# thygate/stable-diffusion-webui-depthmap-script

Measured on NVIDIA H100. Metric: images/sec, higher is better.
Workload: dtype fp16

## Files before the change

stable-diffusion-webui-depthmap-script_b200/csrc/attention_wgmma.cu:

```cuda
#include <cuda.h>
#include <cuda_fp16.h>
#include <math.h>

#include "common.cuh"
#include "tc_common.cuh"

namespace dm {
using namespace tc;

__device__ __forceinline__ float ex2_approx(float x) {
    float y;
    asm("ex2.approx.ftz.f32 %0, %1;" : "=f"(y) : "f"(x));
    return y;
}

int make_tmap_2d(CUtensorMap *tm, const void *ptr, uint64_t rows, uint64_t cols, uint64_t ld, uint32_t box_rows, uint32_t box_cols);

struct AttnParams {
    int B, N, H;
    int C;
    float scale_log2e;
    const __half *bias;
    int bias_ld;
    __half *out;
    const float *rel_table;
    int nrd, gh, gw;
    int sub_stride;
};

constexpr int AT_BQ = 128, AT_BKV = 128, AT_D = 64, AT_STAGES = 2;
constexpr int AT_THREADS = 384;
constexpr int AT_Q_BYTES = AT_BQ * AT_D * 2;
constexpr int AT_KV_BYTES = AT_BKV * AT_D * 2;
constexpr int AT_K_OFF = AT_Q_BYTES;
constexpr int AT_V_OFF = AT_K_OFF + AT_STAGES * AT_KV_BYTES;
constexpr int AT_BAR_OFF = AT_V_OFF + AT_STAGES * AT_KV_BYTES;
constexpr int AT_TAB_OFF = AT_BAR_OFF + 64;
constexpr int AT_SMEM_MAX = 227 * 1024;
constexpr int AT_STAGERS = 96;

static inline int relpos_sub_stride(int gh, int gw) {
    const int span = gh < (AT_BQ - 1) / gw + 2 ? gh : (AT_BQ - 1) / gw + 2;
    return ((2 * span - 1) * (2 * gw - 1) + 1 + 3) & ~3;
}

template <int BIAS_MODE>
__global__ void __launch_bounds__(AT_THREADS, 1) attention_wgmma_kernel(const __grid_constant__ CUtensorMap tmQKV, AttnParams p) {
    extern __shared__ __align__(1024) uint8_t smem_raw[];
    uint8_t *sQ = smem_raw, *sK = smem_raw + AT_K_OFF, *sV = smem_raw + AT_V_OFF;
    uint64_t *bars = reinterpret_cast<uint64_t *>(smem_raw + AT_BAR_OFF);
    uint64_t *q_full = bars, *kv_full = bars + 1, *kv_empty = bars + 1 + AT_STAGES;
    float *s_tab = reinterpret_cast<float *>(smem_raw + AT_TAB_OFF);
    int *s_koff = reinterpret_cast<int *>(s_tab + AT_STAGES * p.sub_stride);

    const int warp = threadIdx.x >> 5, lane = threadIdx.x & 31;
    const int q0 = blockIdx.x * AT_BQ, h = blockIdx.y, b = blockIdx.z;
    const int num_kv = (p.N + AT_BKV - 1) / AT_BKV;
    const int row_base = b * p.N;

    if (threadIdx.x == 0) {
        prefetch_tmap(&tmQKV);
        mbar_init(q_full, 1);
        for (int s = 0; s < AT_STAGES; ++s) {
            mbar_init(&kv_full[s], BIAS_MODE == 2 ? 1 + AT_STAGERS : 1);
            mbar_init(&kv_empty[s], 8);
        }
        fence_barrier_init();
    }
    __syncthreads();

    if (warp < 4) {
        if (threadIdx.x == 0) {
            mbar_arrive_expect_tx(q_full, AT_Q_BYTES);
            tma_load_2d(sQ, &tmQKV, q_full, h * AT_D, row_base + q0);
            for (int j = 0; j < num_kv; ++j) {
                const int s = j % AT_STAGES;
                mbar_wait(&kv_empty[s], ((j / AT_STAGES) & 1) ^ 1);
                mbar_arrive_expect_tx(&kv_full[s], 2 * AT_KV_BYTES);
                tma_load_2d(sK + s * AT_KV_BYTES, &tmQKV, &kv_full[s], p.C + h * AT_D, row_base + j * AT_BKV);
                tma_load_2d(sV + s * AT_KV_BYTES, &tmQKV, &kv_full[s], 2 * p.C + h * AT_D, row_base + j * AT_BKV);
            }
        } else if (BIAS_MODE == 2 && warp >= 1) {
            const int st = threadIdx.x - 32, rw = 2 * p.gw - 1;
            const float *tab = p.rel_table + (size_t)h * p.nrd;
            const int qy_min = (max(q0, 1) - 1) / p.gw, qy_max = (min(q0 + AT_BQ, p.N) - 2) / p.gw;
            for (int j = 0; j < num_kv; ++j) {
                const int s = j % AT_STAGES, kbase = j * AT_BKV;
                const int k_lo = max(kbase, 1), k_hi = min(kbase + AT_BKV, p.N) - 1;
                const int ky_min = (k_lo - 1) / p.gw, ky_max = (k_hi - 1) / p.gw;
                const int lo = (qy_min - ky_max + p.gh - 1) * rw;
                const int cnt = (qy_max - qy_min + ky_max - ky_min + 1) * rw;
                float *sub = s_tab + s * p.sub_stride;
                int *kof = s_koff + s * AT_BKV;
                mbar_wait(&kv_empty[s], ((j / AT_STAGES) & 1) ^ 1);
                for (int i = st; i < cnt; i += AT_STAGERS) sub[i] = __ldg(tab + lo + i);
                if (st == 0) sub[p.sub_stride - 1] = __ldg(tab + p.nrd - 3);
                for (int k = st; k < AT_BKV; k += AT_STAGERS) {
                    const int t = min(max(kbase + k, k_lo), k_hi) - 1;
                    kof[k] = (t / p.gw) * rw + (t % p.gw) + lo;
                }
                mbar_arrive(&kv_full[s]);
            }
        }
        return;
    }

    const int wg = (warp >> 2) - 1, t = lane & 3;
    constexpr float LOG2E = 1.4426950408889634f;
    int qi[2];
    bool q_ok[2];
    const __half *brow[2] = {nullptr, nullptr};
    int rp_base[2] = {0, 0}, rp_mult[2] = {1, 1};
    float rp_k0[2] = {0.f, 0.f};
#pragma unroll
    for (int r = 0; r < 2; ++r) {
        qi[r] = q0 + wg * 64 + (warp & 3) * 16 + (lane >> 2) + 8 * r;
        q_ok[r] = qi[r] < p.N;
        const int qq = q_ok[r] ? qi[r] : 0;
        if (BIAS_MODE == 1) brow[r] = p.bias + ((size_t)h * p.N + qq) * p.bias_ld;
        if (BIAS_MODE == 2) {
            const float *tab = p.rel_table + (size_t)h * p.nrd;
            if (qq == 0) { rp_base[r] = p.sub_stride - 1; rp_mult[r] = 0; rp_k0[r] = __ldg(tab + p.nrd - 1); }
            else {
                const int tt = qq - 1, qy = tt / p.gw, qx = tt % p.gw;
                rp_base[r] = (qy + p.gh - 1) * (2 * p.gw - 1) + (qx + p.gw - 1);
                rp_k0[r] = __ldg(tab + p.nrd - 2);
            }
        }
    }
    float o[32];
#pragma unroll
    for (int i = 0; i < 32; ++i) o[i] = 0.f;
    float m_run[2] = {-INFINITY, -INFINITY}, l_run[2] = {0.f, 0.f};
    const uint64_t qdesc = make_desc_kmajor_sw128(smem_u32(sQ) + wg * (64 * 128));

    mbar_wait(q_full, 0);
    for (int j = 0; j < num_kv; ++j) {
        const int s = j % AT_STAGES;
        const int kbase = j * AT_BKV;
        mbar_wait(&kv_full[s], (j / AT_STAGES) & 1);
        float sc[64];
        const float *sub = s_tab + s * p.sub_stride;
        const int *kof = s_koff + s * AT_BKV;
        const uint64_t kdesc = make_desc_kmajor_sw128(smem_u32(sK + s * AT_KV_BYTES));
        wgmma_fence();
#pragma unroll
        for (int k = 0; k < AT_D / 16; ++k) wgmma_ss<AT_BKV>(sc, qdesc + (uint64_t)(2 * k), kdesc + (uint64_t)(2 * k), k != 0);
        wgmma_commit();
        wgmma_wait<0>();
        float mx[2] = {-INFINITY, -INFINITY};
#pragma unroll
        for (int c = 0; c < AT_BKV / 8; ++c) {
            const int k0 = kbase + 8 * c + 2 * t;
#pragma unroll
            for (int r = 0; r < 2; ++r) {
                float b0 = 0.f, b1 = 0.f;
                if (BIAS_MODE == 1) {
                    const float2 bf = __half22float2(__ldg(reinterpret_cast<const __half2 *>(brow[r] + k0)));
                    b0 = bf.x * LOG2E; b1 = bf.y * LOG2E;
                } else if (BIAS_MODE == 2) {
                    const int2 kk = *reinterpret_cast<const int2 *>(kof + 8 * c + 2 * t);
                    b0 = k0 == 0 ? rp_k0[r] : sub[rp_base[r] - rp_mult[r] * kk.x];
                    b1 = sub[rp_base[r] - rp_mult[r] * kk.y];
                }
                float u0 = fmaf(sc[4 * c + 2 * r], p.scale_log2e, b0), u1 = fmaf(sc[4 * c + 2 * r + 1], p.scale_log2e, b1);
                u0 = k0 < p.N ? u0 : -INFINITY;
                u1 = k0 + 1 < p.N ? u1 : -INFINITY;
                sc[4 * c + 2 * r] = u0; sc[4 * c + 2 * r + 1] = u1;
                mx[r] = fmaxf(mx[r], fmaxf(u0, u1));
            }
        }
        float alpha[2];
#pragma unroll
        for (int r = 0; r < 2; ++r) {
            mx[r] = fmaxf(mx[r], __shfl_xor_sync(0xffffffffu, mx[r], 1));
            mx[r] = fmaxf(mx[r], __shfl_xor_sync(0xffffffffu, mx[r], 2));
            const float m_new = fmaxf(m_run[r], mx[r]);
            alpha[r] = ex2_approx(m_run[r] - m_new);
            m_run[r] = m_new;
        }
        uint32_t pa[AT_BKV / 16][4];
        float ls[2] = {0.f, 0.f};
#pragma unroll
        for (int c = 0; c < AT_BKV / 8; ++c) {
#pragma unroll
            for (int r = 0; r < 2; ++r) {
                const float e0 = ex2_approx(sc[4 * c + 2 * r] - m_run[r]), e1 = ex2_approx(sc[4 * c + 2 * r + 1] - m_run[r]);
                const __half2 h2 = __floats2half2_rn(e0, e1);
                const float2 pr = __half22float2(h2);
                ls[r] += pr.x + pr.y;
                pa[c >> 1][(c & 1) * 2 + r] = *reinterpret_cast<const uint32_t *>(&h2);
            }
        }
#pragma unroll
        for (int r = 0; r < 2; ++r) l_run[r] = fmaf(l_run[r], alpha[r], ls[r]);
#pragma unroll
        for (int c = 0; c < AT_D / 8; ++c) { o[4 * c] *= alpha[0]; o[4 * c + 1] *= alpha[0]; o[4 * c + 2] *= alpha[1]; o[4 * c + 3] *= alpha[1]; }
        const uint32_t sv = smem_u32(sV + s * AT_KV_BYTES);
        wgmma_fence();
#pragma unroll
        for (int k = 0; k < AT_BKV / 16; ++k) wgmma_rs_n64_bt(o, pa[k], make_desc_mnmajor_sw128(sv + k * 16 * 128));
        wgmma_commit();
        wgmma_wait<0>();
        if (lane == 0) mbar_arrive(&kv_empty[s]);
    }
#pragma unroll
    for (int r = 0; r < 2; ++r) {
        float l = l_run[r];
        l += __shfl_xor_sync(0xffffffffu, l, 1);
        l += __shfl_xor_sync(0xffffffffu, l, 2);
        if (!q_ok[r]) continue;
        const float inv = 1.0f / l;
        __half *dst = p.out + (size_t)(row_base + qi[r]) * p.C + h * AT_D + 2 * t;
#pragma unroll
        for (int c = 0; c < AT_D / 8; ++c)
            *reinterpret_cast<__half2 *>(dst + 8 * c) = __floats2half2_rn(o[4 * c + 2 * r] * inv, o[4 * c + 2 * r + 1] * inv);
    }
}

template <int MODE>
static int launch_attn(const CUtensorMap &tm, const AttnParams &p, cudaStream_t stream) {
    const size_t tab = MODE == 2 ? (size_t)AT_STAGES * ((size_t)p.sub_stride * 4 + AT_BKV * 4) : 0;
    if (AT_TAB_OFF + tab > (size_t)AT_SMEM_MAX) { set_error("attention: relative-position window %d x %d too wide for the table sub-windows", p.gh, p.gw); return DM_E_UNSUPPORTED; }
    static PerDeviceFlag configured;
    if (!configured.test_and_set())
        DM_CUDA_CHECK(cudaFuncSetAttribute(attention_wgmma_kernel<MODE>, cudaFuncAttributeMaxDynamicSharedMemorySize, AT_SMEM_MAX));
    dim3 grid((p.N + AT_BQ - 1) / AT_BQ, p.H, p.B);
    attention_wgmma_kernel<MODE><<<grid, AT_THREADS, AT_TAB_OFF + tab, stream>>>(tm, p);
    DM_LAUNCH_CHECK("attention_wgmma_kernel");
    return DM_OK;
}

int attention_f16(const __half *qkv, AttnParams p, cudaStream_t stream, const float *rel_table = nullptr, int nrd = 0, int gh = 0, int gw = 0) {
    if (p.C != p.H * AT_D) { set_error("attention_f16: head_dim must be 64"); return DM_E_UNSUPPORTED; }
    CUtensorMap tm;
    int rc = make_tmap_2d(&tm, qkv, (uint64_t)p.B * p.N, (uint64_t)3 * p.C, (uint64_t)3 * p.C, AT_BQ, AT_D);
    if (rc) return rc;
    if (p.bias && (p.bias_ld % 8 != 0 || p.bias_ld < ((p.N + AT_BKV - 1) / AT_BKV) * AT_BKV)) {
        set_error("attention_f16: bias row pitch must be a multiple of 8 and cover whole 128-key tiles (got %d)", p.bias_ld);
        return DM_E_INVALID;
    }
    p.rel_table = rel_table; p.nrd = nrd; p.gh = gh; p.gw = gw; p.sub_stride = 0;
    if (rel_table) {
        if (gh < 1 || gw < 1 || (long long)gh * gw + 1 != p.N || (long long)nrd != (long long)(2 * gh - 1) * (2 * gw - 1) + 3) {
            set_error("attention_f16: relative-position mode needs N = gh*gw+1 and nrd = (2gh-1)(2gw-1)+3");
            return DM_E_INVALID;
        }
        p.sub_stride = relpos_sub_stride(gh, gw);
        return launch_attn<2>(tm, p, stream);
    }
    return p.bias ? launch_attn<1>(tm, p, stream) : launch_attn<0>(tm, p, stream);
}

}

extern "C" __attribute__((visibility("default"))) int dm_attention_f16(const void *qkv, int B, int N, int H, float scale, const void *bias, int bias_ld,
                                                                    void *out, void *stream) {
    dm::AttnParams p;
    p.B = B; p.N = N; p.H = H; p.C = H * 64;
    p.scale_log2e = scale * 1.4426950408889634f;
    p.bias = (const __half *)bias; p.bias_ld = bias_ld;
    p.out = (__half *)out;
    return dm::attention_f16((const __half *)qkv, p, (cudaStream_t)stream);
}

extern "C" __attribute__((visibility("default"))) int dm_attention_relpos_f16(const void *qkv, int B, int gh, int gw, int H, float scale,
                                                                           const float *rel_table_log2e, int nrd,
                                                                           void *out, void *stream) {
    dm::AttnParams p;
    p.B = B; p.N = gh * gw + 1; p.H = H; p.C = H * 64;
    p.scale_log2e = scale * 1.4426950408889634f;
    p.bias = nullptr; p.bias_ld = 0;
    p.out = (__half *)out;
    if (!rel_table_log2e) { dm::set_error("dm_attention_relpos_f16: table is NULL"); return DM_E_INVALID; }
    return dm::attention_f16((const __half *)qkv, p, (cudaStream_t)stream, rel_table_log2e, nrd, gh, gw);
}
```

stable-diffusion-webui-depthmap-script_b200/csrc/tc_common.cuh:

```cuda
#pragma once
#include <cuda.h>
#include <cuda_fp16.h>
#include <cuda_runtime.h>
#include <stdint.h>

namespace dm {
namespace tc {

__device__ __forceinline__ uint32_t smem_u32(const void *p) { return (uint32_t)__cvta_generic_to_shared(p); }

__device__ __forceinline__ void mbar_init(uint64_t *bar, uint32_t count) {
    asm volatile("mbarrier.init.shared::cta.b64 [%0], %1;" ::"r"(smem_u32(bar)), "r"(count) : "memory");
}
__device__ __forceinline__ void fence_barrier_init() { asm volatile("fence.mbarrier_init.release.cluster;" ::: "memory"); }
__device__ __forceinline__ void fence_proxy_async() { asm volatile("fence.proxy.async.shared::cta;" ::: "memory"); }
__device__ __forceinline__ void mbar_arrive_expect_tx(uint64_t *bar, uint32_t bytes) {
    asm volatile("mbarrier.arrive.expect_tx.shared::cta.b64 _, [%0], %1;" ::"r"(smem_u32(bar)), "r"(bytes) : "memory");
}
__device__ __forceinline__ void mbar_arrive(uint64_t *bar) {
    asm volatile("mbarrier.arrive.shared::cta.b64 _, [%0];" ::"r"(smem_u32(bar)) : "memory");
}
__device__ __forceinline__ bool mbar_try_wait(uint64_t *bar, uint32_t parity) {
    uint32_t done;
    asm volatile(
        "{\n\t.reg .pred p;\n\t"
        "mbarrier.try_wait.parity.shared::cta.b64 p, [%1], %2;\n\t"
        "selp.u32 %0, 1, 0, p;\n\t}"
        : "=r"(done)
        : "r"(smem_u32(bar)), "r"(parity)
        : "memory");
    return done != 0;
}
__device__ __forceinline__ void mbar_wait(uint64_t *bar, uint32_t parity) {
    while (!mbar_try_wait(bar, parity)) {}
}

__device__ __forceinline__ void named_bar_sync(uint32_t id, uint32_t count) {
    asm volatile("bar.sync %0, %1;" ::"r"(id), "r"(count) : "memory");
}
__device__ __forceinline__ void named_bar_arrive(uint32_t id, uint32_t count) {
    asm volatile("bar.arrive %0, %1;" ::"r"(id), "r"(count) : "memory");
}
template <int N>
__device__ __forceinline__ void setmaxnreg_dec() { asm volatile("setmaxnreg.dec.sync.aligned.u32 %0;" ::"n"(N)); }
template <int N>
__device__ __forceinline__ void setmaxnreg_inc() { asm volatile("setmaxnreg.inc.sync.aligned.u32 %0;" ::"n"(N)); }

__device__ __forceinline__ void prefetch_tmap(const CUtensorMap *m) {
    asm volatile("prefetch.tensormap [%0];" ::"l"(reinterpret_cast<uint64_t>(m)) : "memory");
}
__device__ __forceinline__ void tma_load_2d(void *dst, const CUtensorMap *m, uint64_t *bar, int c0, int c1) {
    asm volatile(
        "cp.async.bulk.tensor.2d.shared::cluster.global.mbarrier::complete_tx::bytes [%0], [%1, {%3, %4}], [%2];"
        ::"r"(smem_u32(dst)), "l"(reinterpret_cast<uint64_t>(m)), "r"(smem_u32(bar)), "r"(c0), "r"(c1)
        : "memory");
}
__device__ __forceinline__ void tma_load_4d(void *dst, const CUtensorMap *m, uint64_t *bar, int c0, int c1, int c2, int c3) {
    asm volatile(
        "cp.async.bulk.tensor.4d.shared::cluster.global.mbarrier::complete_tx::bytes [%0], [%1, {%3, %4, %5, %6}], [%2];"
        ::"r"(smem_u32(dst)), "l"(reinterpret_cast<uint64_t>(m)), "r"(smem_u32(bar)), "r"(c0), "r"(c1), "r"(c2), "r"(c3)
        : "memory");
}

__device__ __forceinline__ void wgmma_fence() { asm volatile("wgmma.fence.sync.aligned;" ::: "memory"); }
__device__ __forceinline__ void wgmma_commit() { asm volatile("wgmma.commit_group.sync.aligned;" ::: "memory"); }
template <int N>
__device__ __forceinline__ void wgmma_wait() { asm volatile("wgmma.wait_group.sync.aligned %0;" ::"n"(N) : "memory"); }

template <int N>
__device__ __forceinline__ void wgmma_ss(float (&d)[N / 2], uint64_t adesc, uint64_t bdesc, uint32_t scale_d);
template <>
__device__ __forceinline__ void wgmma_ss<32>(float (&d)[16], uint64_t adesc, uint64_t bdesc, uint32_t scale_d) {
    asm volatile(
        "{\n\t.reg .pred p;\n\t"
        "setp.ne.b32 p, %18, 0;\n\t"
        "wgmma.mma_async.sync.aligned.m64n32k16.f32.f16.f16 "
        "{%0, %1, %2, %3, %4, %5, %6, %7, %8, %9, %10, %11, %12, %13, %14, %15}, "
        "%16, %17, p, 1, 1, 0, 0;\n\t}"
        : "+f"(d[0]), "+f"(d[1]), "+f"(d[2]), "+f"(d[3]), "+f"(d[4]), "+f"(d[5]), "+f"(d[6]), "+f"(d[7]),
          "+f"(d[8]), "+f"(d[9]), "+f"(d[10]), "+f"(d[11]), "+f"(d[12]), "+f"(d[13]), "+f"(d[14]), "+f"(d[15])
        : "l"(adesc), "l"(bdesc), "r"(scale_d)
        : "memory");
}
template <>
__device__ __forceinline__ void wgmma_ss<64>(float (&d)[32], uint64_t adesc, uint64_t bdesc, uint32_t scale_d) {
    asm volatile(
        "{\n\t.reg .pred p;\n\t"
        "setp.ne.b32 p, %34, 0;\n\t"
        "wgmma.mma_async.sync.aligned.m64n64k16.f32.f16.f16 "
        "{%0, %1, %2, %3, %4, %5, %6, %7, %8, %9, %10, %11, %12, %13, %14, %15, %16, %17, %18, %19, %20, %21, %22, %23, %24, %25, %26, %27, %28, %29, %30, %31}, "
        "%32, %33, p, 1, 1, 0, 0;\n\t}"
        : "+f"(d[0]), "+f"(d[1]), "+f"(d[2]), "+f"(d[3]), "+f"(d[4]), "+f"(d[5]), "+f"(d[6]), "+f"(d[7]),
          "+f"(d[8]), "+f"(d[9]), "+f"(d[10]), "+f"(d[11]), "+f"(d[12]), "+f"(d[13]), "+f"(d[14]), "+f"(d[15]),
          "+f"(d[16]), "+f"(d[17]), "+f"(d[18]), "+f"(d[19]), "+f"(d[20]), "+f"(d[21]), "+f"(d[22]), "+f"(d[23]),
          "+f"(d[24]), "+f"(d[25]), "+f"(d[26]), "+f"(d[27]), "+f"(d[28]), "+f"(d[29]), "+f"(d[30]), "+f"(d[31])
        : "l"(adesc), "l"(bdesc), "r"(scale_d)
        : "memory");
}
template <>
__device__ __forceinline__ void wgmma_ss<128>(float (&d)[64], uint64_t adesc, uint64_t bdesc, uint32_t scale_d) {
    asm volatile(
        "{\n\t.reg .pred p;\n\t"
        "setp.ne.b32 p, %66, 0;\n\t"
        "wgmma.mma_async.sync.aligned.m64n128k16.f32.f16.f16 "
        "{%0, %1, %2, %3, %4, %5, %6, %7, %8, %9, %10, %11, %12, %13, %14, %15, %16, %17, %18, %19, %20, %21, %22, %23, %24, %25, %26, %27, %28, %29, %30, %31, %32, %33, %34, %35, %36, %37, %38, %39, %40, %41, %42, %43, %44, %45, %46, %47, %48, %49, %50, %51, %52, %53, %54, %55, %56, %57, %58, %59, %60, %61, %62, %63}, "
        "%64, %65, p, 1, 1, 0, 0;\n\t}"
        : "+f"(d[0]), "+f"(d[1]), "+f"(d[2]), "+f"(d[3]), "+f"(d[4]), "+f"(d[5]), "+f"(d[6]), "+f"(d[7]),
          "+f"(d[8]), "+f"(d[9]), "+f"(d[10]), "+f"(d[11]), "+f"(d[12]), "+f"(d[13]), "+f"(d[14]), "+f"(d[15]),
          "+f"(d[16]), "+f"(d[17]), "+f"(d[18]), "+f"(d[19]), "+f"(d[20]), "+f"(d[21]), "+f"(d[22]), "+f"(d[23]),
          "+f"(d[24]), "+f"(d[25]), "+f"(d[26]), "+f"(d[27]), "+f"(d[28]), "+f"(d[29]), "+f"(d[30]), "+f"(d[31]),
          "+f"(d[32]), "+f"(d[33]), "+f"(d[34]), "+f"(d[35]), "+f"(d[36]), "+f"(d[37]), "+f"(d[38]), "+f"(d[39]),
          "+f"(d[40]), "+f"(d[41]), "+f"(d[42]), "+f"(d[43]), "+f"(d[44]), "+f"(d[45]), "+f"(d[46]), "+f"(d[47]),
          "+f"(d[48]), "+f"(d[49]), "+f"(d[50]), "+f"(d[51]), "+f"(d[52]), "+f"(d[53]), "+f"(d[54]), "+f"(d[55]),
          "+f"(d[56]), "+f"(d[57]), "+f"(d[58]), "+f"(d[59]), "+f"(d[60]), "+f"(d[61]), "+f"(d[62]), "+f"(d[63])
        : "l"(adesc), "l"(bdesc), "r"(scale_d)
        : "memory");
}
template <>
__device__ __forceinline__ void wgmma_ss<256>(float (&d)[128], uint64_t adesc, uint64_t bdesc, uint32_t scale_d) {
    asm volatile(
        "{\n\t.reg .pred p;\n\t"
        "setp.ne.b32 p, %130, 0;\n\t"
        "wgmma.mma_async.sync.aligned.m64n256k16.f32.f16.f16 "
        "{%0, %1, %2, %3, %4, %5, %6, %7, %8, %9, %10, %11, %12, %13, %14, %15, %16, %17, %18, %19, %20, %21, %22, %23, %24, %25, %26, %27, %28, %29, %30, %31, "
        "%32, %33, %34, %35, %36, %37, %38, %39, %40, %41, %42, %43, %44, %45, %46, %47, %48, %49, %50, %51, %52, %53, %54, %55, %56, %57, %58, %59, %60, %61, %62, %63, "
        "%64, %65, %66, %67, %68, %69, %70, %71, %72, %73, %74, %75, %76, %77, %78, %79, %80, %81, %82, %83, %84, %85, %86, %87, %88, %89, %90, %91, %92, %93, %94, %95, "
        "%96, %97, %98, %99, %100, %101, %102, %103, %104, %105, %106, %107, %108, %109, %110, %111, %112, %113, %114, %115, %116, %117, %118, %119, %120, %121, %122, %123, %124, %125, %126, %127}, "
        "%128, %129, p, 1, 1, 0, 0;\n\t}"
        : "+f"(d[0]), "+f"(d[1]), "+f"(d[2]), "+f"(d[3]), "+f"(d[4]), "+f"(d[5]), "+f"(d[6]), "+f"(d[7]),
          "+f"(d[8]), "+f"(d[9]), "+f"(d[10]), "+f"(d[11]), "+f"(d[12]), "+f"(d[13]), "+f"(d[14]), "+f"(d[15]),
          "+f"(d[16]), "+f"(d[17]), "+f"(d[18]), "+f"(d[19]), "+f"(d[20]), "+f"(d[21]), "+f"(d[22]), "+f"(d[23]),
          "+f"(d[24]), "+f"(d[25]), "+f"(d[26]), "+f"(d[27]), "+f"(d[28]), "+f"(d[29]), "+f"(d[30]), "+f"(d[31]),
          "+f"(d[32]), "+f"(d[33]), "+f"(d[34]), "+f"(d[35]), "+f"(d[36]), "+f"(d[37]), "+f"(d[38]), "+f"(d[39]),
          "+f"(d[40]), "+f"(d[41]), "+f"(d[42]), "+f"(d[43]), "+f"(d[44]), "+f"(d[45]), "+f"(d[46]), "+f"(d[47]),
          "+f"(d[48]), "+f"(d[49]), "+f"(d[50]), "+f"(d[51]), "+f"(d[52]), "+f"(d[53]), "+f"(d[54]), "+f"(d[55]),
          "+f"(d[56]), "+f"(d[57]), "+f"(d[58]), "+f"(d[59]), "+f"(d[60]), "+f"(d[61]), "+f"(d[62]), "+f"(d[63]),
          "+f"(d[64]), "+f"(d[65]), "+f"(d[66]), "+f"(d[67]), "+f"(d[68]), "+f"(d[69]), "+f"(d[70]), "+f"(d[71]),
          "+f"(d[72]), "+f"(d[73]), "+f"(d[74]), "+f"(d[75]), "+f"(d[76]), "+f"(d[77]), "+f"(d[78]), "+f"(d[79]),
          "+f"(d[80]), "+f"(d[81]), "+f"(d[82]), "+f"(d[83]), "+f"(d[84]), "+f"(d[85]), "+f"(d[86]), "+f"(d[87]),
          "+f"(d[88]), "+f"(d[89]), "+f"(d[90]), "+f"(d[91]), "+f"(d[92]), "+f"(d[93]), "+f"(d[94]), "+f"(d[95]),
          "+f"(d[96]), "+f"(d[97]), "+f"(d[98]), "+f"(d[99]), "+f"(d[100]), "+f"(d[101]), "+f"(d[102]), "+f"(d[103]),
          "+f"(d[104]), "+f"(d[105]), "+f"(d[106]), "+f"(d[107]), "+f"(d[108]), "+f"(d[109]), "+f"(d[110]), "+f"(d[111]),
          "+f"(d[112]), "+f"(d[113]), "+f"(d[114]), "+f"(d[115]), "+f"(d[116]), "+f"(d[117]), "+f"(d[118]), "+f"(d[119]),
          "+f"(d[120]), "+f"(d[121]), "+f"(d[122]), "+f"(d[123]), "+f"(d[124]), "+f"(d[125]), "+f"(d[126]), "+f"(d[127])
        : "l"(adesc), "l"(bdesc), "r"(scale_d)
        : "memory");
}
__device__ __forceinline__ void wgmma_rs_n64_bt(float (&d)[32], const uint32_t (&a)[4], uint64_t bdesc) {
    asm volatile(
        "wgmma.mma_async.sync.aligned.m64n64k16.f32.f16.f16 "
        "{%0, %1, %2, %3, %4, %5, %6, %7, %8, %9, %10, %11, %12, %13, %14, %15, %16, %17, %18, %19, %20, %21, %22, %23, %24, %25, %26, %27, %28, %29, %30, %31}, "
        "{%32, %33, %34, %35}, %36, 1, 1, 1, 1;"
        : "+f"(d[0]), "+f"(d[1]), "+f"(d[2]), "+f"(d[3]), "+f"(d[4]), "+f"(d[5]), "+f"(d[6]), "+f"(d[7]),
          "+f"(d[8]), "+f"(d[9]), "+f"(d[10]), "+f"(d[11]), "+f"(d[12]), "+f"(d[13]), "+f"(d[14]), "+f"(d[15]),
          "+f"(d[16]), "+f"(d[17]), "+f"(d[18]), "+f"(d[19]), "+f"(d[20]), "+f"(d[21]), "+f"(d[22]), "+f"(d[23]),
          "+f"(d[24]), "+f"(d[25]), "+f"(d[26]), "+f"(d[27]), "+f"(d[28]), "+f"(d[29]), "+f"(d[30]), "+f"(d[31])
        : "r"(a[0]), "r"(a[1]), "r"(a[2]), "r"(a[3]), "l"(bdesc)
        : "memory");
}

__device__ __forceinline__ uint64_t make_desc_kmajor_sw128(uint32_t smem_addr) {
    uint64_t d = 0;
    d |= (uint64_t)((smem_addr >> 4) & 0x3fff);
    d |= (uint64_t)1 << 16;
    d |= (uint64_t)(1024 >> 4) << 32;
    d |= (uint64_t)1 << 62;
    return d;
}
__device__ __forceinline__ uint64_t make_desc_mnmajor_sw128(uint32_t smem_addr) {
    uint64_t d = 0;
    d |= (uint64_t)((smem_addr >> 4) & 0x3fff);
    d |= (uint64_t)(8192 >> 4) << 16;
    d |= (uint64_t)(1024 >> 4) << 32;
    d |= (uint64_t)1 << 62;
    return d;
}

}
}
```

Baseline: 314.2.

## Make attention kernel persistent with ping-pong warpgroups and overlapped PV/QK wgmma

Turns the attention kernel into a persistent kernel whose grid is capped at the SM count and which walks (q-tile, head, batch) tiles. Q is double-buffered and KV gets three stages. The two consumer warpgroups take turns issuing wgmma through named barriers, and each issues the PV product for the previous KV block together with the QK product for the current one. It also adds setmaxnreg register rebalancing, a narrower QK tile for the last partial KV block, and skips masking on blocks that are not the tail. The goal is to hide softmax behind tensor-core work and remove launch and tail overhead, at the cost of more complex synchronisation and higher register pressure.

```diff
diff --git a/stable-diffusion-webui-depthmap-script_b200/csrc/attention_wgmma.cu b/stable-diffusion-webui-depthmap-script_b200/csrc/attention_wgmma.cu
--- a/stable-diffusion-webui-depthmap-script_b200/csrc/attention_wgmma.cu
+++ b/stable-diffusion-webui-depthmap-script_b200/csrc/attention_wgmma.cu
@@ -28,14 +28,14 @@
     int sub_stride;
 };
 
-constexpr int AT_BQ = 128, AT_BKV = 128, AT_D = 64, AT_STAGES = 2;
+constexpr int AT_BQ = 128, AT_BKV = 128, AT_D = 64, AT_STAGES = 3;
 constexpr int AT_THREADS = 384;
 constexpr int AT_Q_BYTES = AT_BQ * AT_D * 2;
 constexpr int AT_KV_BYTES = AT_BKV * AT_D * 2;
-constexpr int AT_K_OFF = AT_Q_BYTES;
+constexpr int AT_K_OFF = 2 * AT_Q_BYTES;
 constexpr int AT_V_OFF = AT_K_OFF + AT_STAGES * AT_KV_BYTES;
 constexpr int AT_BAR_OFF = AT_V_OFF + AT_STAGES * AT_KV_BYTES;
-constexpr int AT_TAB_OFF = AT_BAR_OFF + 64;
+constexpr int AT_TAB_OFF = AT_BAR_OFF + 128;
 constexpr int AT_SMEM_MAX = 227 * 1024;
 constexpr int AT_STAGERS = 96;
 
@@ -44,113 +44,51 @@
     return ((2 * span - 1) * (2 * gw - 1) + 1 + 3) & ~3;
 }
 
+__device__ __forceinline__ void attn_tile(const AttnParams &p, int w, int nq, int &q0, int &h, int &b) {
+    const int hb = w / nq;
+    q0 = (w - hb * nq) * AT_BQ;
+    h = hb % p.H;
+    b = hb / p.H;
+}
+
 template <int BIAS_MODE>
-__global__ void __launch_bounds__(AT_THREADS, 1) attention_wgmma_kernel(const __grid_constant__ CUtensorMap tmQKV, AttnParams p) {
-    extern __shared__ __align__(1024) uint8_t smem_raw[];
-    uint8_t *sQ = smem_raw, *sK = smem_raw + AT_K_OFF, *sV = smem_raw + AT_V_OFF;
-    uint64_t *bars = reinterpret_cast<uint64_t *>(smem_raw + AT_BAR_OFF);
-    uint64_t *q_full = bars, *kv_full = bars + 1, *kv_empty = bars + 1 + AT_STAGES;
-    float *s_tab = reinterpret_cast<float *>(smem_raw + AT_TAB_OFF);
-    int *s_koff = reinterpret_cast<int *>(s_tab + AT_STAGES * p.sub_stride);
-
-    const int warp = threadIdx.x >> 5, lane = threadIdx.x & 31;
-    const int q0 = blockIdx.x * AT_BQ, h = blockIdx.y, b = blockIdx.z;
-    const int num_kv = (p.N + AT_BKV - 1) / AT_BKV;
-    const int row_base = b * p.N;
-
-    if (threadIdx.x == 0) {
-        prefetch_tmap(&tmQKV);
-        mbar_init(q_full, 1);
-        for (int s = 0; s < AT_STAGES; ++s) {
-            mbar_init(&kv_full[s], BIAS_MODE == 2 ? 1 + AT_STAGERS : 1);
-            mbar_init(&kv_empty[s], 8);
-        }
-        fence_barrier_init();
-    }
-    __syncthreads();
-
-    if (warp < 4) {
-        if (threadIdx.x == 0) {
-            mbar_arrive_expect_tx(q_full, AT_Q_BYTES);
-            tma_load_2d(sQ, &tmQKV, q_full, h * AT_D, row_base + q0);
-            for (int j = 0; j < num_kv; ++j) {
-                const int s = j % AT_STAGES;
-                mbar_wait(&kv_empty[s], ((j / AT_STAGES) & 1) ^ 1);
-                mbar_arrive_expect_tx(&kv_full[s], 2 * AT_KV_BYTES);
-                tma_load_2d(sK + s * AT_KV_BYTES, &tmQKV, &kv_full[s], p.C + h * AT_D, row_base + j * AT_BKV);
-                tma_load_2d(sV + s * AT_KV_BYTES, &tmQKV, &kv_full[s], 2 * p.C + h * AT_D, row_base + j * AT_BKV);
-            }
-        } else if (BIAS_MODE == 2 && warp >= 1) {
-            const int st = threadIdx.x - 32, rw = 2 * p.gw - 1;
-            const float *tab = p.rel_table + (size_t)h * p.nrd;
-            const int qy_min = (max(q0, 1) - 1) / p.gw, qy_max = (min(q0 + AT_BQ, p.N) - 2) / p.gw;
-            for (int j = 0; j < num_kv; ++j) {
-                const int s = j % AT_STAGES, kbase = j * AT_BKV;
-                const int k_lo = max(kbase, 1), k_hi = min(kbase + AT_BKV, p.N) - 1;
-                const int ky_min = (k_lo - 1) / p.gw, ky_max = (k_hi - 1) / p.gw;
-                const int lo = (qy_min - ky_max + p.gh - 1) * rw;
-                const int cnt = (qy_max - qy_min + ky_max - ky_min + 1) * rw;
-                float *sub = s_tab + s * p.sub_stride;
-                int *kof = s_koff + s * AT_BKV;
-                mbar_wait(&kv_empty[s], ((j / AT_STAGES) & 1) ^ 1);
-                for (int i = st; i < cnt; i += AT_STAGERS) sub[i] = __ldg(tab + lo + i);
-                if (st == 0) sub[p.sub_stride - 1] = __ldg(tab + p.nrd - 3);
-                for (int k = st; k < AT_BKV; k += AT_STAGERS) {
-                    const int t = min(max(kbase + k, k_lo), k_hi) - 1;
-                    kof[k] = (t / p.gw) * rw + (t % p.gw) + lo;
-                }
-                mbar_arrive(&kv_full[s]);
-            }
-        }
-        return;
-    }
-
-    const int wg = (warp >> 2) - 1, t = lane & 3;
-    constexpr float LOG2E = 1.4426950408889634f;
-    int qi[2];
-    bool q_ok[2];
-    const __half *brow[2] = {nullptr, nullptr};
-    int rp_base[2] = {0, 0}, rp_mult[2] = {1, 1};
-    float rp_k0[2] = {0.f, 0.f};
-#pragma unroll
-    for (int r = 0; r < 2; ++r) {
-        qi[r] = q0 + wg * 64 + (warp & 3) * 16 + (lane >> 2) + 8 * r;
-        q_ok[r] = qi[r] < p.N;
-        const int qq = q_ok[r] ? qi[r] : 0;
-        if (BIAS_MODE == 1) brow[r] = p.bias + ((size_t)h * p.N + qq) * p.bias_ld;
-        if (BIAS_MODE == 2) {
-            const float *tab = p.rel_table + (size_t)h * p.nrd;
-            if (qq == 0) { rp_base[r] = p.sub_stride - 1; rp_mult[r] = 0; rp_k0[r] = __ldg(tab + p.nrd - 1); }
-            else {
-                const int tt = qq - 1, qy = tt / p.gw, qx = tt % p.gw;
-                rp_base[r] = (qy + p.gh - 1) * (2 * p.gw - 1) + (qx + p.gw - 1);
-                rp_k0[r] = __ldg(tab + p.nrd - 2);
-            }
-        }
-    }
+struct AttnRows {
     float o[32];
-#pragma unroll
-    for (int i = 0; i < 32; ++i) o[i] = 0.f;
-    float m_run[2] = {-INFINITY, -INFINITY}, l_run[2] = {0.f, 0.f};
-    const uint64_t qdesc = make_desc_kmajor_sw128(smem_u32(sQ) + wg * (64 * 128));
-
-    mbar_wait(q_full, 0);
-    for (int j = 0; j < num_kv; ++j) {
-        const int s = j % AT_STAGES;
-        const int kbase = j * AT_BKV;
-        mbar_wait(&kv_full[s], (j / AT_STAGES) & 1);
-        float sc[64];
-        const float *sub = s_tab + s * p.sub_stride;
-        const int *kof = s_koff + s * AT_BKV;
-        const uint64_t kdesc = make_desc_kmajor_sw128(smem_u32(sK + s * AT_KV_BYTES));
-        wgmma_fence();
-#pragma unroll
-        for (int k = 0; k < AT_D / 16; ++k) wgmma_ss<AT_BKV>(sc, qdesc + (uint64_t)(2 * k), kdesc + (uint64_t)(2 * k), k != 0);
-        wgmma_commit();
-        wgmma_wait<0>();
+    float m_run[2], l_run[2];
+    uint32_t pa[AT_BKV / 16][4];
+    const __half *brow[2];
+    int rp_base[2], rp_mult[2];
+    float rp_k0[2];
+
+    __device__ __forceinline__ void init(const AttnParams &p, const int (&qi)[2], int h) {
+#pragma unroll
+        for (int i = 0; i < 32; ++i) o[i] = 0.f;
+#pragma unroll
+        for (int r = 0; r < 2; ++r) {
+            m_run[r] = -INFINITY; l_run[r] = 0.f;
+            brow[r] = nullptr; rp_base[r] = 0; rp_mult[r] = 1; rp_k0[r] = 0.f;
+            const int qq = qi[r] < p.N ? qi[r] : 0;
+            if (BIAS_MODE == 1) brow[r] = p.bias + ((size_t)h * p.N + qq) * p.bias_ld;
+            if (BIAS_MODE == 2) {
+                const float *tab = p.rel_table + (size_t)h * p.nrd;
+                if (qq == 0) { rp_base[r] = p.sub_stride - 1; rp_mult[r] = 0; rp_k0[r] = __ldg(tab + p.nrd - 1); }
+                else {
+                    const int tt = qq - 1, qy = tt / p.gw, qx = tt % p.gw;
+                    rp_base[r] = (qy + p.gh - 1) * (2 * p.gw - 1) + (qx + p.gw - 1);
+                    rp_k0[r] = __ldg(tab + p.nrd - 2);
+                }
+            }
+        }
+    }
+
+    template <int TN, bool TAIL>
+    __device__ __forceinline__ void scores(float (&sc)[TN / 2], const AttnParams &p, int kbase, int t, const float *sub,
+                                           const int *kof, float (&alpha)[2]) {
+        constexpr float LOG2E = 1.4426950408889634f;
+        const bool key0 = kbase == 0 && t == 0;
         float mx[2] = {-INFINITY, -INFINITY};
 #pragma unroll
-        for (int c = 0; c < AT_BKV / 8; ++c) {
+        for (int c = 0; c < TN / 8; ++c) {
             const int k0 = kbase + 8 * c + 2 * t;
 #pragma unroll
             for (int r = 0; r < 2; ++r) {
@@ -160,17 +98,18 @@
                     b0 = bf.x * LOG2E; b1 = bf.y * LOG2E;
                 } else if (BIAS_MODE == 2) {
                     const int2 kk = *reinterpret_cast<const int2 *>(kof + 8 * c + 2 * t);
-                    b0 = k0 == 0 ? rp_k0[r] : sub[rp_base[r] - rp_mult[r] * kk.x];
+                    b0 = (c == 0 && key0) ? rp_k0[r] : sub[rp_base[r] - rp_mult[r] * kk.x];
                     b1 = sub[rp_base[r] - rp_mult[r] * kk.y];
                 }
                 float u0 = fmaf(sc[4 * c + 2 * r], p.scale_log2e, b0), u1 = fmaf(sc[4 * c + 2 * r + 1], p.scale_log2e, b1);
-                u0 = k0 < p.N ? u0 : -INFINITY;
-                u1 = k0 + 1 < p.N ? u1 : -INFINITY;
+                if (TAIL) {
+                    u0 = k0 < p.N ? u0 : -INFINITY;
+                    u1 = k0 + 1 < p.N ? u1 : -INFINITY;
+                }
                 sc[4 * c + 2 * r] = u0; sc[4 * c + 2 * r + 1] = u1;
                 mx[r] = fmaxf(mx[r], fmaxf(u0, u1));
             }
         }
-        float alpha[2];
 #pragma unroll
         for (int r = 0; r < 2; ++r) {
             mx[r] = fmaxf(mx[r], __shfl_xor_sync(0xffffffffu, mx[r], 1));
@@ -179,14 +118,23 @@
             alpha[r] = ex2_approx(m_run[r] - m_new);
             m_run[r] = m_new;
         }
-        uint32_t pa[AT_BKV / 16][4];
+#pragma unroll
+        for (int c = 0; c < TN / 8; ++c)
+#pragma unroll
+            for (int r = 0; r < 2; ++r) {
+                sc[4 * c + 2 * r] = ex2_approx(sc[4 * c + 2 * r] - m_run[r]);
+                sc[4 * c + 2 * r + 1] = ex2_approx(sc[4 * c + 2 * r + 1] - m_run[r]);
+            }
+    }
+
+    template <int TN>
+    __device__ __forceinline__ void pack(const float (&sc)[TN / 2], const float (&alpha)[2]) {
         float ls[2] = {0.f, 0.f};
 #pragma unroll
-        for (int c = 0; c < AT_BKV / 8; ++c) {
+        for (int c = 0; c < TN / 8; ++c) {
 #pragma unroll
             for (int r = 0; r < 2; ++r) {
-                const float e0 = ex2_approx(sc[4 * c + 2 * r] - m_run[r]), e1 = ex2_approx(sc[4 * c + 2 * r + 1] - m_run[r]);
-                const __half2 h2 = __floats2half2_rn(e0, e1);
+                const __half2 h2 = __floats2half2_rn(sc[4 * c + 2 * r], sc[4 * c + 2 * r + 1]);
                 const float2 pr = __half22float2(h2);
                 ls[r] += pr.x + pr.y;
                 pa[c >> 1][(c & 1) * 2 + r] = *reinterpret_cast<const uint32_t *>(&h2);
@@ -196,25 +144,209 @@
         for (int r = 0; r < 2; ++r) l_run[r] = fmaf(l_run[r], alpha[r], ls[r]);
 #pragma unroll
         for (int c = 0; c < AT_D / 8; ++c) { o[4 * c] *= alpha[0]; o[4 * c + 1] *= alpha[0]; o[4 * c + 2] *= alpha[1]; o[4 * c + 3] *= alpha[1]; }
-        const uint32_t sv = smem_u32(sV + s * AT_KV_BYTES);
-        wgmma_fence();
-#pragma unroll
-        for (int k = 0; k < AT_BKV / 16; ++k) wgmma_rs_n64_bt(o, pa[k], make_desc_mnmajor_sw128(sv + k * 16 * 128));
+    }
+
+    template <int SLICES>
+    __device__ __forceinline__ void issue_pv(uint32_t sv) {
+#pragma unroll
+        for (int k = 0; k < SLICES; ++k) wgmma_rs_n64_bt(o, pa[k], make_desc_mnmajor_sw128(sv + k * 16 * 128));
         wgmma_commit();
+    }
+};
+
+__device__ __forceinline__ void turn_begin(int wg) { named_bar_sync(1 + wg, 256); }
+__device__ __forceinline__ void turn_end(int wg, bool last) {
+    if (!(last && wg == 1)) named_bar_arrive(2 - wg, 256);
+}
+
+template <int BIAS_MODE, int TN, bool TAIL, bool PREV>
+__device__ __forceinline__ void attn_step(AttnRows<BIAS_MODE> &st, const AttnParams &p, int wg, int j, int t, uint64_t qdesc,
+                                          uint32_t sk, uint32_t sv_prev, const float *sub, const int *kof, uint64_t *empty_prev,
+                                          int lane) {
+    float sc[TN / 2];
+    float alpha[2];
+    const uint64_t kdesc = make_desc_kmajor_sw128(sk);
+    reg_fence(st.pa);
+    reg_fence(st.o);
+    turn_begin(wg);
+    wgmma_fence();
+#pragma unroll
+    for (int k = 0; k < AT_D / 16; ++k) wgmma_ss<TN>(sc, qdesc + (uint64_t)(2 * k), kdesc + (uint64_t)(2 * k), k != 0);
+    wgmma_commit();
+    if (PREV) st.template issue_pv<AT_BKV / 16>(sv_prev);
+    turn_end(wg, false);
+    if (PREV) wgmma_wait<1>();
+    else wgmma_wait<0>();
+    reg_fence(sc);
+    st.template scores<TN, TAIL>(sc, p, j * AT_BKV, t, sub, kof, alpha);
+    if (PREV) {
         wgmma_wait<0>();
-        if (lane == 0) mbar_arrive(&kv_empty[s]);
-    }
-#pragma unroll
-    for (int r = 0; r < 2; ++r) {
-        float l = l_run[r];
-        l += __shfl_xor_sync(0xffffffffu, l, 1);
-        l += __shfl_xor_sync(0xffffffffu, l, 2);
-        if (!q_ok[r]) continue;
-        const float inv = 1.0f / l;
-        __half *dst = p.out + (size_t)(row_base + qi[r]) * p.C + h * AT_D + 2 * t;
-#pragma unroll
-        for (int c = 0; c < AT_D / 8; ++c)
-            *reinterpret_cast<__half2 *>(dst + 8 * c) = __floats2half2_rn(o[4 * c + 2 * r] * inv, o[4 * c + 2 * r + 1] * inv);
+        reg_fence(st.o);
+        if (lane == 0) mbar_arrive(empty_prev);
+    }
+    st.template pack<TN>(sc, alpha);
+}
+
+template <int BIAS_MODE, int TN, bool TAIL, bool PREV>
+__device__ __forceinline__ void attn_last(AttnRows<BIAS_MODE> &st, const AttnParams &p, int wg, int j, int t, uint64_t qdesc,
+                                          uint32_t sk, uint32_t sv_prev, uint32_t sv, const float *sub, const int *kof,
+                                          uint64_t *empty_prev, int lane, bool last_tile) {
+    attn_step<BIAS_MODE, TN, TAIL, PREV>(st, p, wg, j, t, qdesc, sk, sv_prev, sub, kof, empty_prev, lane);
+    reg_fence(st.pa);
+    reg_fence(st.o);
+    turn_begin(wg);
+    wgmma_fence();
+    st.template issue_pv<TN / 16>(sv);
+    turn_end(wg, last_tile);
+    wgmma_wait<0>();
+    reg_fence(st.o);
+}
+
+template <int BIAS_MODE>
+__global__ void __launch_bounds__(AT_THREADS, 1) attention_wgmma_kernel(const __grid_constant__ CUtensorMap tmQKV, AttnParams p) {
+    extern __shared__ __align__(1024) uint8_t smem_raw[];
+    uint8_t *sQ = smem_raw, *sK = smem_raw + AT_K_OFF, *sV = smem_raw + AT_V_OFF;
+    uint64_t *bars = reinterpret_cast<uint64_t *>(smem_raw + AT_BAR_OFF);
+    uint64_t *q_full = bars, *q_empty = bars + 2, *kv_full = bars + 4, *kv_empty = bars + 4 + AT_STAGES;
+    float *s_tab = reinterpret_cast<float *>(smem_raw + AT_TAB_OFF);
+    int *s_koff = reinterpret_cast<int *>(s_tab + AT_STAGES * p.sub_stride);
+
+    const int warp = threadIdx.x >> 5, lane = threadIdx.x & 31;
+    const int nq = (p.N + AT_BQ - 1) / AT_BQ;
+    const int num_kv = (p.N + AT_BKV - 1) / AT_BKV;
+    const int my_tiles = (nq * p.H * p.B - (int)blockIdx.x + (int)gridDim.x - 1) / (int)gridDim.x;
+
+    if (threadIdx.x == 0) {
+        prefetch_tmap(&tmQKV);
+        for (int i = 0; i < 2; ++i) { mbar_init(&q_full[i], 1); mbar_init(&q_empty[i], 8); }
+        for (int s = 0; s < AT_STAGES; ++s) {
+            mbar_init(&kv_full[s], BIAS_MODE == 2 ? 1 + AT_STAGERS : 1);
+            mbar_init(&kv_empty[s], 8);
+        }
+        fence_barrier_init();
+    }
+    __syncthreads();
+
+    if (warp < 4) {
+        setmaxnreg_dec<56>();
+        if (threadIdx.x == 0) {
+            int stage = 0, phase = 0;
+            for (int i = 0; i < my_tiles; ++i) {
+                int q0, h, b;
+                attn_tile(p, blockIdx.x + i * gridDim.x, nq, q0, h, b);
+                const int row_base = b * p.N, qb = i & 1;
+                mbar_wait(&q_empty[qb], ((i >> 1) & 1) ^ 1);
+                mbar_arrive_expect_tx(&q_full[qb], AT_Q_BYTES);
+                tma_load_2d(sQ + qb * AT_Q_BYTES, &tmQKV, &q_full[qb], h * AT_D, row_base + q0);
+                for (int j = 0; j < num_kv; ++j) {
+                    mbar_wait(&kv_empty[stage], phase ^ 1);
+                    mbar_arrive_expect_tx(&kv_full[stage], 2 * AT_KV_BYTES);
+                    tma_load_2d(sK + stage * AT_KV_BYTES, &tmQKV, &kv_full[stage], p.C + h * AT_D, row_base + j * AT_BKV);
+                    tma_load_2d(sV + stage * AT_KV_BYTES, &tmQKV, &kv_full[stage], 2 * p.C + h * AT_D, row_base + j * AT_BKV);
+                    if (++stage == AT_STAGES) { stage = 0; phase ^= 1; }
+                }
+            }
+        } else if (BIAS_MODE == 2 && warp >= 1) {
+            const int st = threadIdx.x - 32, rw = 2 * p.gw - 1;
+            int stage = 0, phase = 0;
+            for (int i = 0; i < my_tiles; ++i) {
+                int q0, h, b;
+                attn_tile(p, blockIdx.x + i * gridDim.x, nq, q0, h, b);
+                const float *tab = p.rel_table + (size_t)h * p.nrd;
+                const int qy_min = (max(q0, 1) - 1) / p.gw, qy_max = (min(q0 + AT_BQ, p.N) - 2) / p.gw;
+                for (int j = 0; j < num_kv; ++j) {
+                    const int kbase = j * AT_BKV;
+                    const int k_lo = max(kbase, 1), k_hi = min(kbase + AT_BKV, p.N) - 1;
+                    const int ky_min = (k_lo - 1) / p.gw, ky_max = (k_hi - 1) / p.gw;
+                    const int lo = (qy_min - ky_max + p.gh - 1) * rw;
+                    const int cnt = (qy_max - qy_min + ky_max - ky_min + 1) * rw;
+                    float *sub = s_tab + stage * p.sub_stride;
+                    int *kof = s_koff + stage * AT_BKV;
+                    mbar_wait(&kv_empty[stage], phase ^ 1);
+                    for (int k = st; k < cnt; k += AT_STAGERS) sub[k] = __ldg(tab + lo + k);
+                    if (st == 0) sub[p.sub_stride - 1] = __ldg(tab + p.nrd - 3);
+                    for (int k = st; k < AT_BKV; k += AT_STAGERS) {
+                        const int tk = min(max(kbase + k, k_lo), k_hi) - 1;
+                        kof[k] = (tk / p.gw) * rw + (tk % p.gw) + lo;
+                    }
+                    mbar_arrive(&kv_full[stage]);
+                    if (++stage == AT_STAGES) { stage = 0; phase ^= 1; }
+                }
+            }
+        }
+        return;
+    }
+
+    setmaxnreg_inc<224>();
+    const int wg = (warp >> 2) - 1, t = lane & 3;
+    const int tail = p.N - (num_kv - 1) * AT_BKV;
+    const int tn = tail == AT_BKV ? 0 : (tail <= 16 ? 16 : (tail <= 32 ? 32 : (tail <= 64 ? 64 : 128)));
+    int stage = 0, phase = 0;
+    if (wg == 1) named_bar_arrive(1, 256);
+    for (int i = 0; i < my_tiles; ++i) {
+        int q0, h, b;
+        attn_tile(p, blockIdx.x + i * gridDim.x, nq, q0, h, b);
+        const bool last_tile = i + 1 == my_tiles;
+        const int qb = i & 1;
+        mbar_wait(&q_full[qb], (i >> 1) & 1);
+        if (q0 + 64 * wg >= p.N) {
+            for (int j = 0; j < num_kv; ++j) {
+                mbar_wait(&kv_full[stage], phase);
+                turn_begin(wg);
+                turn_end(wg, false);
+                if (lane == 0) mbar_arrive(&kv_empty[stage]);
+                if (++stage == AT_STAGES) { stage = 0; phase ^= 1; }
+            }
+            turn_begin(wg);
+            turn_end(wg, last_tile);
+        } else {
+            int qi[2];
+#pragma unroll
+            for (int r = 0; r < 2; ++r) qi[r] = q0 + wg * 64 + (warp & 3) * 16 + (lane >> 2) + 8 * r;
+            AttnRows<BIAS_MODE> st;
+            st.init(p, qi, h);
+            const uint64_t qdesc = make_desc_kmajor_sw128(smem_u32(sQ + qb * AT_Q_BYTES) + wg * (64 * 128));
+            int prev = stage;
+            mbar_wait(&kv_full[stage], phase);
+            const float *sub = s_tab + stage * p.sub_stride;
+            const int *kof = s_koff + stage * AT_BKV;
+            uint32_t sk = smem_u32(sK + stage * AT_KV_BYTES), sv = smem_u32(sV + stage * AT_KV_BYTES);
+            if (num_kv == 1) {
+                attn_last<BIAS_MODE, AT_BKV, true, false>(st, p, wg, 0, t, qdesc, sk, sv, sv, sub, kof, nullptr, lane, last_tile);
+            } else {
+                attn_step<BIAS_MODE, AT_BKV, false, false>(st, p, wg, 0, t, qdesc, sk, sv, sub, kof, nullptr, lane);
+                for (int j = 1; j < num_kv; ++j) {
+                    if (++stage == AT_STAGES) { stage = 0; phase ^= 1; }
+                    mbar_wait(&kv_full[stage], phase);
+                    const uint32_t sv_prev = smem_u32(sV + prev * AT_KV_BYTES);
+                    sk = smem_u32(sK + stage * AT_KV_BYTES); sv = smem_u32(sV + stage * AT_KV_BYTES);
+                    sub = s_tab + stage * p.sub_stride;
+                    kof = s_koff + stage * AT_BKV;
+                    if (j + 1 < num_kv) attn_step<BIAS_MODE, AT_BKV, false, true>(st, p, wg, j, t, qdesc, sk, sv_prev, sub, kof, &kv_empty[prev], lane);
+                    else if (tn == 0) attn_last<BIAS_MODE, AT_BKV, false, true>(st, p, wg, j, t, qdesc, sk, sv_prev, sv, sub, kof, &kv_empty[prev], lane, last_tile);
+                    else if (tn == 16) attn_last<BIAS_MODE, 16, true, true>(st, p, wg, j, t, qdesc, sk, sv_prev, sv, sub, kof, &kv_empty[prev], lane, last_tile);
+                    else if (tn == 32) attn_last<BIAS_MODE, 32, true, true>(st, p, wg, j, t, qdesc, sk, sv_prev, sv, sub, kof, &kv_empty[prev], lane, last_tile);
+                    else if (tn == 64) attn_last<BIAS_MODE, 64, true, true>(st, p, wg, j, t, qdesc, sk, sv_prev, sv, sub, kof, &kv_empty[prev], lane, last_tile);
+                    else attn_last<BIAS_MODE, AT_BKV, true, true>(st, p, wg, j, t, qdesc, sk, sv_prev, sv, sub, kof, &kv_empty[prev], lane, last_tile);
+                    prev = stage;
+                }
+            }
+            if (lane == 0) mbar_arrive(&kv_empty[stage]);
+            if (++stage == AT_STAGES) { stage = 0; phase ^= 1; }
+#pragma unroll
+            for (int r = 0; r < 2; ++r) {
+                float l = st.l_run[r];
+                l += __shfl_xor_sync(0xffffffffu, l, 1);
+                l += __shfl_xor_sync(0xffffffffu, l, 2);
+                if (qi[r] >= p.N) continue;
+                const float inv = 1.0f / l;
+                __half *dst = p.out + (size_t)(b * p.N + qi[r]) * p.C + h * AT_D + 2 * t;
+#pragma unroll
+                for (int c = 0; c < AT_D / 8; ++c)
+                    *reinterpret_cast<__half2 *>(dst + 8 * c) = __floats2half2_rn(st.o[4 * c + 2 * r] * inv, st.o[4 * c + 2 * r + 1] * inv);
+            }
+        }
+        if (lane == 0) mbar_arrive(&q_empty[qb]);
     }
 }
 
@@ -223,9 +355,11 @@
     const size_t tab = MODE == 2 ? (size_t)AT_STAGES * ((size_t)p.sub_stride * 4 + AT_BKV * 4) : 0;
     if (AT_TAB_OFF + tab > (size_t)AT_SMEM_MAX) { set_error("attention: relative-position window %d x %d too wide for the table sub-windows", p.gh, p.gw); return DM_E_UNSUPPORTED; }
     static PerDeviceFlag configured;
+    static PerDeviceAttr sms(cudaDevAttrMultiProcessorCount);
     if (!configured.test_and_set())
         DM_CUDA_CHECK(cudaFuncSetAttribute(attention_wgmma_kernel<MODE>, cudaFuncAttributeMaxDynamicSharedMemorySize, AT_SMEM_MAX));
-    dim3 grid((p.N + AT_BQ - 1) / AT_BQ, p.H, p.B);
+    const int tiles = (p.N + AT_BQ - 1) / AT_BQ * p.H * p.B;
+    const int grid = tiles < sms.get() ? tiles : sms.get();
     attention_wgmma_kernel<MODE><<<grid, AT_THREADS, AT_TAB_OFF + tab, stream>>>(tm, p);
     DM_LAUNCH_CHECK("attention_wgmma_kernel");
     return DM_OK;
diff --git a/stable-diffusion-webui-depthmap-script_b200/csrc/tc_common.cuh b/stable-diffusion-webui-depthmap-script_b200/csrc/tc_common.cuh
--- a/stable-diffusion-webui-depthmap-script_b200/csrc/tc_common.cuh
+++ b/stable-diffusion-webui-depthmap-script_b200/csrc/tc_common.cuh
@@ -66,9 +66,33 @@
 __device__ __forceinline__ void wgmma_commit() { asm volatile("wgmma.commit_group.sync.aligned;" ::: "memory"); }
 template <int N>
 __device__ __forceinline__ void wgmma_wait() { asm volatile("wgmma.wait_group.sync.aligned %0;" ::"n"(N) : "memory"); }
+template <int N>
+__device__ __forceinline__ void reg_fence(float (&r)[N]) {
+#pragma unroll
+    for (int i = 0; i < N; ++i) asm volatile("" : "+f"(r[i])::"memory");
+}
+template <int M, int N>
+__device__ __forceinline__ void reg_fence(uint32_t (&r)[M][N]) {
+#pragma unroll
+    for (int i = 0; i < M; ++i)
+#pragma unroll
+        for (int k = 0; k < N; ++k) asm volatile("" : "+r"(r[i][k])::"memory");
+}
 
 template <int N>
 __device__ __forceinline__ void wgmma_ss(float (&d)[N / 2], uint64_t adesc, uint64_t bdesc, uint32_t scale_d);
+template <>
+__device__ __forceinline__ void wgmma_ss<16>(float (&d)[8], uint64_t adesc, uint64_t bdesc, uint32_t scale_d) {
+    asm volatile(
+        "{\n\t.reg .pred p;\n\t"
+        "setp.ne.b32 p, %10, 0;\n\t"
+        "wgmma.mma_async.sync.aligned.m64n16k16.f32.f16.f16 "
+        "{%0, %1, %2, %3, %4, %5, %6, %7}, "
+        "%8, %9, p, 1, 1, 0, 0;\n\t}"
+        : "+f"(d[0]), "+f"(d[1]), "+f"(d[2]), "+f"(d[3]), "+f"(d[4]), "+f"(d[5]), "+f"(d[6]), "+f"(d[7])
+        : "l"(adesc), "l"(bdesc), "r"(scale_d)
+        : "memory");
+}
 template <>
 __device__ __forceinline__ void wgmma_ss<32>(float (&d)[16], uint64_t adesc, uint64_t bdesc, uint32_t scale_d) {
     asm volatile(
```

After: 323.3 (median of 6 runs). +2.9%, better.
